# revdotcom/paper_accurate_fast_cheap

Hardware: AMD Instinct MI355X
Metric: audio-sec/sec (1/RTF) GigaSpeech long-form encode (higher is better)
Workload: dtype f32+bf16-slot

## Files before the change

### paper_accurate_fast_cheap_amd/csrc/gemm_ph.hip

```cpp
#include <climits>
#include <cstdlib>
#include <cstring>
#include <type_traits>

#include "pafc_common.h"
#include "../../include/pafc_encoder_ops.h"

namespace pafc {
namespace {

struct PhParams {
    const bf16_t *A, *W;
    const void *bias;
    const void *res;
    void *out;
    long M;
    int N, K;
    long lda, ldw, ldo, ldr;
    long sA, sW, sO, sB, sR;
    float alpha;
    int mtiles, ntiles;
    int tm;
    int batch;
    int nk1, pb_shift;
    long pb_bytes;
    int nsteps, a_lo, w_lo;
    int w_step;
    long lo_off;
    float *ln_stats;
    const float *ln_csum;
    float ln_eps, ln_inv_c;
    int T1, F1, T2, F2, Ci, CiA, CiW, spt, inv_spt;
    long in_bytes;
#ifdef PH_STAMPS
    unsigned long long *stamps;
#endif
};

#ifdef PH_STAMPS
#define PH_STAMP(i) do { if (stamp_on) st[(i)] = __builtin_amdgcn_s_memtime(); } while (0)
#else
#define PH_STAMP(i) do { } while (0)
#endif

__device__ __forceinline__ void dma16(__amdgpu_buffer_rsrc_t rsrc, unsigned lane_off, unsigned uniform_off, void *lds_wave_base) {
    __builtin_amdgcn_raw_ptr_buffer_load_lds(rsrc, (__attribute__((address_space(3))) void *)lds_wave_base, 16, lane_off,
                                             uniform_off, 0, 0);
}
__device__ __forceinline__ __amdgpu_buffer_rsrc_t make_rsrc(const void *base, long bytes) {
    return __builtin_amdgcn_make_buffer_rsrc(const_cast<void *>(base), 0, (int)(bytes > 0x7fffffffL ? 0x7fffffffL : bytes), 0x00020000);
}

#ifndef PH_ST_AUX
#define PH_ST_AUX 0
#endif
#define PH_WAIT(N) asm volatile("s_waitcnt vmcnt(" #N ")" ::: "memory")
template <int N>
__device__ __forceinline__ void wait_vm() {
    static_assert(N >= 0 && N < 64, "vmcnt is a 6-bit counter");
    asm volatile("s_waitcnt vmcnt(%0)" ::"n"(N) : "memory");
}

constexpr int PBN = 256, PBK = 64;
constexpr unsigned PH_OOB = 0xC0000000u;

template <bool GLU, int ACT, int RES, int OUT, bool CONV = false, int LNF = 0, bool SPL = false, bool KSL = false>
__global__ __launch_bounds__(512, 2) void gemm_ph_kernel(const PhParams p) {
    constexpr int BN = PBN;
    constexpr int UA = 128 * 128;
    constexpr int UB = (BN / 2) * 128;
    constexpr int STEP = 2 * UA + 2 * UB;
    constexpr int OFF_A0 = 0, OFF_A1 = UA, OFF_B0 = 2 * UA, OFF_B1 = 2 * UA + UB;
    constexpr int TN = 2;
    constexpr int DA = UA / 8192;
    constexpr int DB = UB / 8192;
    constexpr int OSZ = OUT == 1 ? 4 : 2;
    constexpr bool BIASF32 = OUT != 0;
    constexpr int NST = 8 * (GLU ? 1 : 2) * (OUT == 0 ? 1 : 2) + (LNF == 2 ? 8 : 0);
    static_assert(LNF == 0 || (OUT == 0 && !CONV), "LayerNorm folding: bf16 GEMMs");
    static_assert(!SPL || LNF == 0, "shared-fragment split operands: not with a folded LayerNorm");
    static_assert(LNF != 1 || (RES == 0 && (GLU || ACT == 1)), "LNF 1: the w_1 (SiLU) / pointwise_conv1 (GLU) projections");
    static_assert(LNF != 2 || RES == 1, "LNF 2: a residual GEMM");
    static_assert(!(GLU && (ACT != 0 || RES != 0)), "GLU excludes an activation and a residual");
    static_assert(!(RES != 0 && ACT != 0), "the layer never pairs a residual with an activation");
    static_assert(!KSL || (SPL && !CONV && !GLU && ACT == 0 && RES == 0 && OUT == 1), "K slices: fp32 partial products of split operands");
    extern __shared__ __attribute__((aligned(1024))) unsigned char lds[];

    const int tid = threadIdx.x, lane = tid & 63;
    const int wave = __builtin_amdgcn_readfirstlane(tid >> 6);
    const int wr = wave >> 2, wc = wave & 3;
    const long nblk = (long)p.mtiles * p.ntiles;
    const long total = nblk * p.batch;
    const long per = total / 8;
    const int nt = SPL ? p.nsteps : p.K / PBK;

    auto pix_off = [&](long m) -> long {
        const long tf = (long)p.T2 * p.F2;
        const long bb = m / tf, rem = m - bb * tf;
        const long t2 = rem / p.F2, f2 = rem - t2 * p.F2;
        return (((bb * p.T1 + 2 * t2) * p.F1 + 2 * f2) * p.CiA) * 2;
    };

    struct Tile {
        long m0;
        int n0, z, vr;
        __amdgpu_buffer_rsrc_t Ar, Wr;
    };
    auto make_tile = [&](long t, Tile &T) {
        const bool real = t < total;
        long tt = real ? t : 0;
        if (tt < per * 8) tt = (tt % 8) * per + tt / 8;
        T.z = (int)(tt / nblk);
        const long bid = tt % nblk;
        const int mt0 = (int)(bid / p.ntiles), nt0 = (int)(bid % p.ntiles);
        T.m0 = (long)mt0 * p.tm;
        T.n0 = nt0 * BN;
        T.vr = (int)min((long)p.tm, p.M - T.m0);
        if constexpr (CONV) {
            const long a_base = pix_off(T.m0);
            T.Ar = make_rsrc(reinterpret_cast<const unsigned char *>(p.A) + a_base, real ? p.in_bytes - a_base : 0);
            T.Wr = make_rsrc(p.W + (long)T.n0 * p.CiW, real ? ((long)8 * p.N + p.N - T.n0) * p.CiW * 2 : 0);
        } else {
            T.Ar = make_rsrc(p.A + T.z * p.sA + T.m0 * p.lda, real ? (p.M - T.m0) * p.lda * 2 : 0);
            T.Wr = make_rsrc(p.W + T.z * p.sW + (long)T.n0 * p.ldw, real ? ((long)(p.N - 1 - T.n0) * p.ldw + p.K) * 2 : 0);
        }
    };

    unsigned a_off[2][DA], b_off[2][DB];
    auto a_offsets = [&](const Tile &T, int h) {
        int sl = lane;
        asm volatile("" : "+v"(sl));
        const int sub = sl >> 3, pch = sl & 7;
#pragma unroll
        for (int j = 0; j < DA; ++j) {
            const int u = (wave * DA + j) * 8 + sub;
            const int row = (u >> 6) * 128 + h * 64 + (u & 63);
            const int sc = pch ^ sub;
            const unsigned coff = SPL ? (unsigned)(16 * (sc & 3) + (sc >> 2) * p.a_lo) : (unsigned)(16 * sc);
            a_off[h][j] = CONV ? (unsigned)(pix_off(T.m0 + row) - pix_off(T.m0)) + coff
                               : (unsigned)((long)row * p.lda * 2) + coff;
        }
    };
    auto b_offsets = [&]() {
        const int sub = lane >> 3, pch = lane & 7;
#pragma unroll
        for (int h = 0; h < 2; ++h)
#pragma unroll
            for (int j = 0; j < DB; ++j) {
                const int u = (wave * DB + j) * 8 + sub;
                const int r = u & 31;
                const int pc = ((r & 15) >> 2) * 8 + (r >> 4) * 4 + (r & 3);
                const int sc = pch ^ sub;
                const unsigned coff = SPL ? (unsigned)(16 * (sc & 3) + (sc >> 2) * p.w_lo) : (unsigned)(16 * sc);
                b_off[h][j] = (unsigned)((long)((u >> 5) * 64 + h * 32 + pc) * (CONV ? p.CiW : p.ldw) * 2) + coff;
            }
    };
    auto a_soff = [&](int kt) -> unsigned {
        if constexpr (SPL && !CONV) {
            const int blk = kt >> p.pb_shift, c = kt - (blk << p.pb_shift);
            return (unsigned)(blk * 2 * p.pb_bytes + c * 64);
        } else if constexpr (SPL) {
            const int tap = (kt * p.inv_spt) >> 16, kc = kt - tap * p.spt;
            const int dt = (tap * 11) >> 5, df = tap - 3 * dt;
            return (unsigned)(((dt * p.F1 + df) * p.CiA) * 2 + kc * 64);
        } else if constexpr (!CONV) {
            const int seg = (kt >= p.nk1) + (kt >= 2 * p.nk1);
            const int r = kt - seg * p.nk1;
            const int blk = r >> p.pb_shift, c = r - (blk << p.pb_shift);
            return (unsigned)(blk * 2 * p.pb_bytes + (seg == 1 ? p.pb_bytes : 0) + c * 128);
        } else {
            const int tap = (kt * p.inv_spt) >> 16, kc = kt - tap * p.spt;
            const int seg = (kc >= p.nk1) + (kc >= 2 * p.nk1), cc = kc - seg * p.nk1;
            const int dt = (tap * 11) >> 5, df = tap - 3 * dt;
            return (unsigned)(((dt * p.F1 + df) * p.CiA + (seg == 1 ? p.Ci : 0)) * 2 + cc * 128);
        }
    };
    auto w_soff = [&](int kt) -> unsigned {
        if constexpr (!CONV) return SPL ? kt * p.w_step : kt * 128;
        const int tap = (kt * p.inv_spt) >> 16, kc = kt - tap * p.spt;
        return (unsigned)(tap * p.N * p.CiW * 2 + kc * (SPL ? 64 : 128));
    };
    auto stage_a = [&](const Tile &T, int h, int buf, int kt) {
#ifdef PH_ABL_NODMA
        return;
#endif
        if constexpr (KSL) kt += T.z * nt;
#pragma unroll
        for (int j = 0; j < DA; ++j)
            dma16(T.Ar, a_off[h][j], a_soff(kt), lds + buf * STEP + (h ? OFF_A1 : OFF_A0) + (wave * DA + j) * 1024);
    };
    auto stage_b = [&](const Tile &T, int h, int buf, int kt) {
#ifdef PH_ABL_NODMA
        return;
#endif
        if constexpr (KSL) kt += T.z * nt;
#pragma unroll
        for (int j = 0; j < DB; ++j)
            dma16(T.Wr, b_off[h][j], w_soff(kt), lds + buf * STEP + (h ? OFF_B1 : OFF_B0) + (wave * DB + j) * 1024);
    };

    const int fr = lane & 15, kq = lane >> 4;
    const unsigned frag = fr * 128 + ((kq ^ (fr & 7)) * 16);
    const unsigned la = wr * (64 * 128) + frag;
    const unsigned lb = wc * (32 * 128) + frag;

    bf16x8 af[4][2], bf0[TN][2], bf1[TN][2];
    auto read_a = [&](int h, int buf) {
#ifdef PH_ABL_NOREAD
        return;
#endif
        const unsigned char *base = lds + buf * STEP + (h ? OFF_A1 : OFF_A0);
#pragma unroll
        for (int i = 0; i < 4; ++i) {
            af[i][0] = *reinterpret_cast<const bf16x8 *>(base + la + i * 2048);
            af[i][1] = *reinterpret_cast<const bf16x8 *>(base + (la ^ 64) + i * 2048);
        }
    };
    auto read_b = [&](int h, int buf, bf16x8 (&dst)[TN][2]) {
#ifdef PH_ABL_NOREAD
        return;
#endif
        const unsigned char *base = lds + buf * STEP + (h ? OFF_B1 : OFF_B0);
#pragma unroll
        for (int j = 0; j < TN; ++j) {
            dst[j][0] = *reinterpret_cast<const bf16x8 *>(base + lb + j * 2048);
            dst[j][1] = *reinterpret_cast<const bf16x8 *>(base + (lb ^ 64) + j * 2048);
        }
    };

    Tile cur, nxt;
    make_tile(blockIdx.x, cur);
    a_offsets(cur, 0);
    a_offsets(cur, 1);
    b_offsets();
    stage_a(cur, 0, 0, 0); stage_b(cur, 0, 0, 0); stage_b(cur, 1, 0, 0); stage_a(cur, 1, 0, 0);
    stage_a(cur, 0, 1, 1); stage_b(cur, 0, 1, 1);
    __builtin_amdgcn_sched_barrier(0);
    wait_vm<8>();
    __builtin_amdgcn_sched_barrier(0);
    bool first = true;

    for (long t = blockIdx.x; t < total; t += gridDim.x) {
#ifdef PH_STAMPS
    const bool stamp_on = (wave == 0 || wave == 4) && lane == 0 && cur.z == 0;
    unsigned long long *st = p.stamps + ((size_t)t * 2 + (wave >> 2)) * 64;
    PH_STAMP(0);
#endif
    make_tile(CONV ? total : t + gridDim.x, nxt);
    if constexpr (CONV) {
        if (!first) {
            a_offsets(cur, 0);
            a_offsets(cur, 1);
            stage_a(cur, 0, 0, 0); stage_b(cur, 0, 0, 0); stage_b(cur, 1, 0, 0); stage_a(cur, 1, 0, 0);
            stage_a(cur, 0, 1, 1); stage_b(cur, 0, 1, 1);
            __builtin_amdgcn_sched_barrier(0);
            wait_vm<8>();
            __builtin_amdgcn_sched_barrier(0);
        }
    }
    const bool after_stores = !CONV && !first;
    const bool half_on[2] = {wr * 128 < cur.vr, wr * 128 + 64 < cur.vr};
    constexpr int NBL = LNF == 1 ? 4 : 1;
    {
        const long esz = BIASF32 ? 4 : 2;
        const __amdgpu_buffer_rsrc_t Br = make_rsrc(reinterpret_cast<const unsigned char *>(p.bias) + ((long)cur.z * p.sB + cur.n0) * esz,
                                                    p.bias ? (long)(p.N - cur.n0) * esz : 0);
        dma16(Br, lane * 16, 0, lds + 2 * STEP + wave * 1024);
        if constexpr (LNF == 1) {
            const __amdgpu_buffer_rsrc_t Cr = make_rsrc(p.ln_csum + cur.n0, (long)(p.N - cur.n0) * 4);
            dma16(Cr, lane * 16, 0, lds + 2 * STEP + 8 * 1024 + wave * 1024);
        }
    }

    f32x4 acc[2][2][4][TN];
#pragma unroll
    for (int a = 0; a < 2; ++a)
#pragma unroll
        for (int b = 0; b < 2; ++b)
#pragma unroll
            for (int i = 0; i < 4; ++i)
#pragma unroll
                for (int j = 0; j < TN; ++j) acc[a][b][i][j] = f32x4{0.f, 0.f, 0.f, 0.f};

    auto mma = [&](int mi, int nj, const bf16x8 (&bqf)[TN][2]) {
        __builtin_amdgcn_s_setprio(1);
#ifdef PH_ABL_NOMFMA
        if (false) {
#else
        if (half_on[mi]) {
#endif
            if constexpr (SPL) {
#pragma unroll
                for (int pr = 0; pr < 3; ++pr)
#pragma unroll
                    for (int i = 0; i < 4; ++i)
#pragma unroll
                        for (int j = 0; j < TN; ++j)
                            acc[mi][nj][i][j] = __builtin_amdgcn_mfma_f32_16x16x32_bf16(bqf[j][pr == 2], af[i][pr == 1], acc[mi][nj][i][j], 0, 0, 0);
            } else {
#pragma unroll
                for (int ks = 0; ks < 2; ++ks)
#pragma unroll
                    for (int i = 0; i < 4; ++i)
#pragma unroll
                        for (int j = 0; j < TN; ++j)
                            acc[mi][nj][i][j] = __builtin_amdgcn_mfma_f32_16x16x32_bf16(bqf[j][ks], af[i][ks], acc[mi][nj][i][j], 0, 0, 0);
            }
        }
        __builtin_amdgcn_s_setprio(0);
    };

#ifdef PH_ABL_NOBAR
#define PH_BAR1() do { } while (0)
#else
#define PH_BAR1() __builtin_amdgcn_s_barrier()
#endif
#ifdef PH_ABL_NOEND
#define PH_BAR2() do { } while (0)
#else
#define PH_BAR2() __builtin_amdgcn_s_barrier()
#endif
#define PH_SYNC()                                                                  \
    do {                                                                           \
        if (kt == 0) { if (after_stores) wait_vm<8 + NST + NBL>(); else wait_vm<8 + NBL>(); } \
        else wait_vm<8>();                                                         \
        PH_BAR1();                                                                 \
        __builtin_amdgcn_sched_barrier(0);                                         \
    } while (0)
#define PH_END()                                                                   \
    do {                                                                           \
        __builtin_amdgcn_sched_barrier(0);                                         \
        PH_BAR2();                                                                 \
        __builtin_amdgcn_sched_barrier(0);                                         \
    } while (0)

    auto kstep = [&](auto parc, int kt) {
        constexpr int PAR = decltype(parc)::value;
        const int last = nt - 1 - kt;
        read_b(0, PAR, bf0);
        read_a(0, PAR);
        if (last >= 1) stage_b(cur, 1, PAR ^ 1, kt + 1);
        else stage_b(nxt, 1, PAR ^ 1, 0);
        PH_SYNC();
        mma(0, 0, bf0);
        PH_END();
        read_b(1, PAR, bf1);
        if (last >= 1) stage_a(cur, 1, PAR ^ 1, kt + 1);
        else stage_a(nxt, 1, PAR ^ 1, 0);
        PH_SYNC();
        mma(0, 1, bf1);
        PH_END();
        read_a(1, PAR);
        if (last >= 2) stage_a(cur, 0, PAR, kt + 2);
        else stage_a(nxt, 0, PAR, 1 - last);
        PH_SYNC();
        mma(1, 1, bf1);
        PH_END();
        if (last >= 2) stage_b(cur, 0, PAR, kt + 2);
        else stage_b(nxt, 0, PAR, 1 - last);
        PH_SYNC();
        mma(1, 0, bf0);
        PH_END();
    };
    using I0 = std::integral_constant<int, 0>;
    using I1 = std::integral_constant<int, 1>;

    __builtin_amdgcn_s_barrier();
    if constexpr (LNF == 1) {
        const __amdgpu_buffer_rsrc_t Sd = make_rsrc(p.ln_stats + (cur.z * p.M + cur.m0) * 16, (p.M - cur.m0) * 64);
#pragma unroll
        for (int j = 0; j < 2; ++j)
            dma16(Sd, (wave * 2 + j) * 1024 + lane * 16, 0, lds + 2 * STEP + 16 * 1024 + (wave * 2 + j) * 1024);
    }
    if (wr == 1) __builtin_amdgcn_s_barrier();
    PH_STAMP(1);

    for (int kt = 0; kt < nt; kt += 2) {
        kstep(I0{}, kt);
        PH_STAMP(2 + (kt < 40 ? kt : 40));
        kstep(I1{}, kt + 1);
        PH_STAMP(3 + (kt < 40 ? kt : 40));
    }
    if (wr == 0) __builtin_amdgcn_s_barrier();
    PH_STAMP(50);
#undef PH_SYNC
#undef PH_END

    int etid = tid;
    asm volatile("" : "+v"(etid));
    const int efr = etid & 15, ekq = (etid >> 4) & 3;
    const int ncol = GLU ? p.N / 2 : p.N;
    const int nrt = (cur.vr + 15) >> 4;
    const __amdgpu_buffer_rsrc_t Or = make_rsrc(reinterpret_cast<unsigned char *>(p.out) + (cur.z * p.sO + cur.m0 * p.ldo) * OSZ,
                                                ((p.M - 1 - cur.m0) * p.ldo + (OUT == 2 ? p.lo_off : 0) + ncol) * OSZ);
    constexpr int RSZ = RES == 2 ? 4 : 2;
    __amdgpu_buffer_rsrc_t Rr = Or;
    if constexpr (RES != 0)
        Rr = make_rsrc(reinterpret_cast<const unsigned char *>(p.res) + (cur.z * p.sR + cur.m0 * p.ldr) * RSZ,
                       ((p.M - 1 - cur.m0) * p.ldr + p.N) * RSZ);
    const bool has_bias = p.bias != nullptr;
    auto bias8 = [&](int nj, float (&f)[8]) {
        const unsigned char *slot = lds + 2 * STEP + wave * 1024 + (wc * 64 + nj * 32 + ekq * 8) * (BIASF32 ? 4 : 2);
        if (!has_bias) {
#pragma unroll
            for (int e = 0; e < 8; ++e) f[e] = 0.f;
        } else if constexpr (BIASF32) {
            const u32x4 q0 = *reinterpret_cast<const u32x4 *>(slot), q1 = *reinterpret_cast<const u32x4 *>(slot + 16);
            f[0] = __uint_as_float(q0.x); f[1] = __uint_as_float(q0.y); f[2] = __uint_as_float(q0.z); f[3] = __uint_as_float(q0.w);
            f[4] = __uint_as_float(q1.x); f[5] = __uint_as_float(q1.y); f[6] = __uint_as_float(q1.z); f[7] = __uint_as_float(q1.w);
        } else {
            Elem<bf16_t>::unpack(*reinterpret_cast<const u32x4 *>(slot), f);
        }
    };
    auto store8 = [&](const float (&o)[8], bool live, int row, int col) {
        const bool ok = row < cur.vr && col < ncol;
        const unsigned off = ok ? (unsigned)(((long)row * p.ldo + col) * OSZ) : PH_OOB;
        if constexpr (OUT == 0) {
            u32x4 w{0u, 0u, 0u, 0u};
            if (live) w = u32x4{pack_bf16_rne(o[0], o[1]), pack_bf16_rne(o[2], o[3]), pack_bf16_rne(o[4], o[5]), pack_bf16_rne(o[6], o[7])};
            __builtin_amdgcn_raw_buffer_store_b128(w, Or, off, 0, PH_ST_AUX);
        } else if constexpr (OUT == 1) {
            u32x4 w0{0u, 0u, 0u, 0u}, w1{0u, 0u, 0u, 0u};
            if (live) {
                w0 = u32x4{__float_as_uint(o[0]), __float_as_uint(o[1]), __float_as_uint(o[2]), __float_as_uint(o[3])};
                w1 = u32x4{__float_as_uint(o[4]), __float_as_uint(o[5]), __float_as_uint(o[6]), __float_as_uint(o[7])};
            }
            __builtin_amdgcn_raw_buffer_store_b128(w0, Or, off, 0, PH_ST_AUX);
            __builtin_amdgcn_raw_buffer_store_b128(w1, Or, ok ? off + 16 : PH_OOB, 0, PH_ST_AUX);
        } else {
            u32x4 wh{0u, 0u, 0u, 0u}, wl{0u, 0u, 0u, 0u};
            if (live) {
                float lo[8], hf[8];
                wh = u32x4{pack_bf16_rne(o[0], o[1]), pack_bf16_rne(o[2], o[3]), pack_bf16_rne(o[4], o[5]), pack_bf16_rne(o[6], o[7])};
                Elem<bf16_t>::unpack(wh, hf);
#pragma unroll
                for (int e = 0; e < 8; ++e) lo[e] = o[e] - hf[e];
                wl = u32x4{pack_bf16_rne(lo[0], lo[1]), pack_bf16_rne(lo[2], lo[3]), pack_bf16_rne(lo[4], lo[5]),
                           pack_bf16_rne(lo[6], lo[7])};
            }
            __builtin_amdgcn_raw_buffer_store_b128(wh, Or, off, 0, PH_ST_AUX);
            __builtin_amdgcn_raw_buffer_store_b128(wl, Or, ok ? off + (unsigned)(p.lo_off * 2) : PH_OOB, 0, PH_ST_AUX);
        }
    };
    __amdgpu_buffer_rsrc_t Sr = Or;
    if constexpr (LNF == 2) Sr = make_rsrc(p.ln_stats + (cur.z * p.M + cur.m0) * 16, (p.M - cur.m0) * 64);
    auto row_read = [&](int g, u32x4 (&v)[4]) {
        const unsigned char *rp = lds + 2 * STEP + 16 * 1024 + (wr * 128 + g * 16 + efr) * 64;
#pragma unroll
        for (int q = 0; q < 4; ++q) v[q] = *reinterpret_cast<const u32x4 *>(rp + q * 16);
    };
    auto row_norm = [&](const u32x4 (&v)[4], float &rstd, float &nm) {
        float s1 = 0.f, s2 = 0.f;
#pragma unroll
        for (int q = 0; q < 4; ++q) {
            s1 += __uint_as_float(v[q].x) + __uint_as_float(v[q].z);
            s2 += __uint_as_float(v[q].y) + __uint_as_float(v[q].w);
        }
        const float mean = s1 * p.ln_inv_c;
        const float var = fmaxf(fmaf(-mean, mean, s2 * p.ln_inv_c), 0.f);
        rstd = rsqrtf(var + p.ln_eps);
        nm = -mean * rstd;
    };
    auto csum8 = [&](int nj, float (&f)[8]) {
        const unsigned char *slot = lds + 2 * STEP + 8 * 1024 + wave * 1024 + (wc * 64 + nj * 32 + ekq * 8) * 4;
        const u32x4 q0 = *reinterpret_cast<const u32x4 *>(slot), q1 = *reinterpret_cast<const u32x4 *>(slot + 16);
        f[0] = __uint_as_float(q0.x); f[1] = __uint_as_float(q0.y); f[2] = __uint_as_float(q0.z); f[3] = __uint_as_float(q0.w);
        f[4] = __uint_as_float(q1.x); f[5] = __uint_as_float(q1.y); f[6] = __uint_as_float(q1.z); f[7] = __uint_as_float(q1.w);
    };
    constexpr int RLD = RES == 2 ? 2 : 1;
    float lcs[LNF == 1 ? 2 : 1][8], lbv[LNF == 1 ? 2 : 1][8], nx_rstd = 1.f, nx_nm = 0.f;
    if constexpr (LNF == 1) {
        csum8(0, lcs[0]); csum8(LNF == 1 ? 1 : 0, lcs[LNF == 1 ? 1 : 0]);
        bias8(0, lbv[0]); bias8(LNF == 1 ? 1 : 0, lbv[LNF == 1 ? 1 : 0]);
        u32x4 v0[4];
        row_read(0, v0);
        row_norm(v0, nx_rstd, nx_nm);
    }
    float gst1[LNF == 2 ? 8 : 1], gst2[LNF == 2 ? 8 : 1];
#pragma unroll
    for (int mi = 0; mi < 2; ++mi) {
        u32x4 rr[RES != 0 ? 4 : 1][2][RLD];
        if constexpr (RES != 0) {
            __builtin_amdgcn_sched_barrier(0);
#pragma unroll
            for (int i = 0; i < 4; ++i)
#pragma unroll
                for (int nj = 0; nj < 2; ++nj) {
                    const int row = wr * 128 + mi * 64 + i * 16 + efr, col = cur.n0 + wc * 64 + nj * 32 + ekq * 8;
                    const bool ok = row < cur.vr && col < p.N;
                    const unsigned off = ok ? (unsigned)(((long)row * p.ldr + col) * RSZ) : PH_OOB;
#pragma unroll
                    for (int q = 0; q < RLD; ++q) rr[i][nj][q] = __builtin_amdgcn_raw_buffer_load_b128(Rr, ok ? off + 16 * q : PH_OOB, 0, 0);
                }
        }
#pragma unroll
        for (int i = 0; i < 4; ++i) {
            __builtin_amdgcn_sched_barrier(0);
            const int g = mi * 4 + i;
            const bool live = wr * 8 + g < nrt;
            const int row = wr * 128 + g * 16 + efr;
            const float ln_rstd = nx_rstd, ln_nm = nx_nm;
            u32x4 vn[4];
            if constexpr (LNF == 1) row_read(g < 7 ? g + 1 : 7, vn);
            if constexpr (GLU) {
                float o[8];
                if (live) {
                    float bv[8], bg[8];
                    if constexpr (LNF == 1) {
#pragma unroll
                        for (int e = 0; e < 8; ++e) {
                            bv[e] = fmaf(ln_nm, lcs[0][e], lbv[0][e]);
                            bg[e] = fmaf(ln_nm, lcs[LNF == 1 ? 1 : 0][e], lbv[LNF == 1 ? 1 : 0][e]);
                        }
                    } else {
                        bias8(0, bv);
                        bias8(1, bg);
                    }
                    const float sc = LNF == 1 ? ln_rstd : p.alpha;
#pragma unroll
                    for (int j = 0; j < TN; ++j)
#pragma unroll
                        for (int e = 0; e < 4; ++e) {
                            const float a = fmaf(acc[mi][0][i][j][e], sc, bv[j * 4 + e]);
                            const float b = fmaf(acc[mi][1][i][j][e], sc, bg[j * 4 + e]);
                            o[j * 4 + e] = a * __builtin_amdgcn_rcpf(1.f + __expf(-b));
                        }
                }
                store8(o, live, row, cur.n0 / 2 + wc * 32 + ekq * 8);
            } else {
                float st1 = 0.f, st2 = 0.f;
#pragma unroll
                for (int nj = 0; nj < 2; ++nj) {
                    const int col = cur.n0 + wc * 64 + nj * 32 + ekq * 8;
                    float o[8];
                    if (live) {
                        float bv[8];
                        if constexpr (LNF == 1) {
#pragma unroll
                            for (int e = 0; e < 8; ++e) bv[e] = fmaf(ln_nm, lcs[LNF == 1 ? nj : 0][e], lbv[LNF == 1 ? nj : 0][e]);
                        } else {
                            bias8(nj, bv);
                        }
                        const float sc = LNF == 1 ? ln_rstd : p.alpha;
#pragma unroll
                        for (int j = 0; j < TN; ++j)
#pragma unroll
                            for (int e = 0; e < 4; ++e)
                                o[j * 4 + e] = epilogue_act<ACT>(fmaf(acc[mi][nj][i][j][e], sc, bv[j * 4 + e]));
                        if constexpr (RES == 1) {
                            float rv[8];
                            Elem<bf16_t>::unpack(rr[i][nj][0], rv);
#pragma unroll
                            for (int e = 0; e < 8; ++e) o[e] += rv[e];
                        } else if constexpr (RES == 2) {
                            o[0] += __uint_as_float(rr[i][nj][0].x); o[1] += __uint_as_float(rr[i][nj][0].y);
                            o[2] += __uint_as_float(rr[i][nj][0].z); o[3] += __uint_as_float(rr[i][nj][0].w);
                            o[4] += __uint_as_float(rr[i][nj][RLD - 1].x); o[5] += __uint_as_float(rr[i][nj][RLD - 1].y);
                            o[6] += __uint_as_float(rr[i][nj][RLD - 1].z); o[7] += __uint_as_float(rr[i][nj][RLD - 1].w);
                        }
                        if constexpr (LNF == 2) {
                            float q[8];
                            Elem<bf16_t>::unpack(u32x4{pack_bf16_rne(o[0], o[1]), pack_bf16_rne(o[2], o[3]), pack_bf16_rne(o[4], o[5]),
                                                       pack_bf16_rne(o[6], o[7])}, q);
#pragma unroll
                            for (int e = 0; e < 8; ++e) { st1 += q[e]; st2 = fmaf(q[e], q[e], st2); }
                        }
                    }
                    store8(o, live, row, col);
                }
                if constexpr (LNF == 2) { gst1[LNF == 2 ? g : 0] = live ? st1 : 0.f; gst2[LNF == 2 ? g : 0] = live ? st2 : 0.f; }
            }
            if constexpr (LNF == 1) row_norm(vn, nx_rstd, nx_nm);
        }
    }
    if constexpr (LNF == 2) {
        __builtin_amdgcn_sched_barrier(0);
#pragma unroll
        for (int g = 0; g < 8; ++g) { gst1[g] += __shfl_xor(gst1[g], 16, 64); gst2[g] += __shfl_xor(gst2[g], 16, 64); }
#pragma unroll
        for (int g = 0; g < 8; ++g) { gst1[g] += __shfl_xor(gst1[g], 32, 64); gst2[g] += __shfl_xor(gst2[g], 32, 64); }
#pragma unroll
        for (int g = 0; g < 8; ++g) {
            const int row = wr * 128 + g * 16 + efr;
            const bool ok = ekq == 0 && row < cur.vr;
            const unsigned off = ok ? (unsigned)(row * 64 + ((cur.n0 >> 8) * 4 + wc) * 8) : PH_OOB;
            __builtin_amdgcn_raw_buffer_store_b64(u32x2{__float_as_uint(gst1[g]), __float_as_uint(gst2[g])}, Sr, off, 0, 0);
        }
    }
    __builtin_amdgcn_sched_barrier(0);
    first = false;
    if constexpr (CONV) make_tile(t + gridDim.x, cur);
    else cur = nxt;
    PH_STAMP(53);
    }
    PH_WAIT(0);
}

__global__ __launch_bounds__(256) void gemm_ph_ktail_fixup_kernel(const float *__restrict__ part, long slab, int kslices,
                                                                  const float *__restrict__ bias, const float *res, long ldr,
                                                                  float *out, long ldo, long rows, int N, float alpha) {
    const int nq = N >> 2;
    const long total = rows * nq;
    for (long i = (long)blockIdx.x * blockDim.x + threadIdx.x; i < total; i += (long)gridDim.x * blockDim.x) {
        const long m = i / nq;
        const int n = (int)(i - m * nq) << 2;
        float4 acc = *reinterpret_cast<const float4 *>(part + m * N + n);
        for (int z = 1; z < kslices; ++z) {
            const float4 q = *reinterpret_cast<const float4 *>(part + z * slab + m * N + n);
            acc.x += q.x; acc.y += q.y; acc.z += q.z; acc.w += q.w;
        }
        float4 b = make_float4(0.f, 0.f, 0.f, 0.f);
        if (bias) b = *reinterpret_cast<const float4 *>(bias + n);
        float4 o = make_float4(fmaf(acc.x, alpha, b.x), fmaf(acc.y, alpha, b.y), fmaf(acc.z, alpha, b.z), fmaf(acc.w, alpha, b.w));
        if (res) {
            const float4 r = *reinterpret_cast<const float4 *>(res + m * ldr + n);
            o.x += r.x; o.y += r.y; o.z += r.z; o.w += r.w;
        }
        *reinterpret_cast<float4 *>(out + m * ldo + n) = o;
    }
}

template <bool GLU, int ACT, int RES, int OUT, bool CONV = false, int LNF = 0, bool SPL = false, bool KSL = false>
int launch_ph(const PhParams &p, int batch, hipStream_t s) {
    constexpr size_t lds = 2 * (2 * 128 * 128 + 2 * (PBN / 2) * 128) + 8 * 1024 + (LNF == 1 ? 8 * 1024 + 16 * 1024 : 0);
    auto kern = gemm_ph_kernel<GLU, ACT, RES, OUT, CONV, LNF, SPL, KSL>;
    static bool attr_set[64];
    int dev = 0;
    if (hipGetDevice(&dev) != hipSuccess) return PAFC_ERR_LAUNCH;
    if (dev < 0 || dev >= 64 || !attr_set[dev]) {
        if (hipFuncSetAttribute((const void *)kern, hipFuncAttributeMaxDynamicSharedMemorySize, (int)lds) != hipSuccess)
            return PAFC_ERR_LAUNCH;
        if (dev >= 0 && dev < 64) attr_set[dev] = true;
    }
    const int cus = device_cus();
    PhParams q = p;
    q.batch = batch;
    const long total = (long)p.mtiles * p.ntiles * batch;
    const long grid = total < cus ? total : cus;
    hipLaunchKernelGGL(kern, dim3((unsigned)grid), dim3(512), lds, s, q);
    return hipGetLastError() == hipSuccess ? PAFC_OK : PAFC_ERR_LAUNCH;
}

int g_split_walk = -1;
bool split_shared_fragments() {
    if (g_split_walk < 0) {
        const char *e = getenv("PAFC_SPLIT_WALK");
        g_split_walk = !(e && std::strcmp(e, "hilohi") == 0);
    }
    return g_split_walk != 0;
}

}
}

extern "C" int pafc_gemm_ph_ex(long M, int N, int K, int batch, const void *A, long lda, long strideA, int a_split, const void *W,
                               long ldw, long strideW, const void *bias, long strideBias, const void *residual, int res_kind,
                               long ldr, long strideR, void *out, int out_kind, long ldo, long lo_off, long strideO, float alpha,
                               int act, int tile_m, pafc_stream_t stream) {
    return pafc_gemm_ph_ex2(M, N, K, batch, A, lda, strideA, a_split, 0, W, ldw, strideW, bias, strideBias, residual, res_kind, ldr,
                            strideR, out, out_kind, ldo, lo_off, strideO, alpha, act, tile_m, stream);
}

extern "C" int pafc_gemm_ph_ex2(long M, int N, int K, int batch, const void *A, long lda, long strideA, int a_split,
                                int a_plane_block, const void *W, long ldw, long strideW, const void *bias, long strideBias,
                                const void *residual, int res_kind, long ldr, long strideR, void *out, int out_kind, long ldo,
                                long lo_off, long strideO, float alpha, int act, int tile_m, pafc_stream_t stream) {
    if (!A || !W || !out) return PAFC_ERR_NULL_POINTER;
    if (M <= 0 || N <= 0 || K <= 0 || batch <= 0 || batch > 65535) return PAFC_ERR_BAD_DIMS;
    if (act < 0 || act > 4 || out_kind < 0 || out_kind > 2 || res_kind < 0 || res_kind > 2) return PAFC_ERR_UNSUPPORTED;
    if (!residual) res_kind = 0;
    else if (res_kind == 0) return PAFC_ERR_BAD_DIMS;
    const bool glu = act == 4;
    if (tile_m < 64 || tile_m > 256 || tile_m % 64) return PAFC_ERR_UNSUPPORTED;
    if (N % 8 || K % 128) return PAFC_ERR_UNSUPPORTED;
    if (glu && (N % 256 || residual)) return PAFC_ERR_UNSUPPORTED;
    if (residual && act != 0) return PAFC_ERR_UNSUPPORTED;
    if (res_kind == 1 && out_kind != 0) return PAFC_ERR_UNSUPPORTED;
    if (res_kind == 2 && out_kind != 1) return PAFC_ERR_UNSUPPORTED;
    const int Kw = a_split ? 3 * K : K;
    const int No = glu ? N / 2 : N;
    if (lda < (a_split ? 2 * K : K) || ldw < Kw || (residual && ldr < N)) return PAFC_ERR_BAD_DIMS;
    if (out_kind == 2 ? (lo_off < No || ldo < lo_off + No) : ldo < No) return PAFC_ERR_BAD_DIMS;
    if ((lda | ldw | strideA | strideW) % 8 || (ldo | strideO | lo_off) % 8 || (residual && ((ldr | strideR) % 8))) return PAFC_ERR_ALIGNMENT;
    if ((((uintptr_t)A | (uintptr_t)W | (uintptr_t)out | (uintptr_t)residual | (uintptr_t)bias) & 15) != 0) return PAFC_ERR_ALIGNMENT;
    if ((double)M * lda * 2 >= 2.0e9 || (double)N * ldw * 2 >= 2.0e9) return PAFC_ERR_UNSUPPORTED;
    if ((double)256 * ldo * 4 >= 2.0e9 || (residual && (double)256 * ldr * 4 >= 2.0e9)) return PAFC_ERR_UNSUPPORTED;
    pafc::PhParams p{};
    p.A = (const pafc::bf16_t *)A; p.W = (const pafc::bf16_t *)W; p.bias = bias; p.res = residual; p.out = out;
    p.M = M; p.N = N; p.K = Kw;
    p.lda = lda; p.ldw = ldw; p.ldo = ldo; p.ldr = ldr;
    p.sA = strideA; p.sW = strideW; p.sO = strideO; p.sB = strideBias; p.sR = strideR;
    p.alpha = alpha;
    p.nk1 = a_split ? K / 64 : INT_MAX / 4;
    p.pb_shift = 31;
    p.pb_bytes = (long)K * 2;
    if (a_split && a_plane_block) {
        int sh = 0;
        while ((64 << sh) < a_plane_block) ++sh;
        if ((64 << sh) != a_plane_block || K % a_plane_block) return PAFC_ERR_UNSUPPORTED;
        p.pb_shift = sh;
        p.pb_bytes = (long)a_plane_block * 2;
    }
    p.lo_off = lo_off;
    p.tm = tile_m;
    p.mtiles = (int)((M + tile_m - 1) / tile_m);
    p.ntiles = (N + 255) / 256;
    if ((long)p.mtiles * p.ntiles > 0x7fffffffL) return PAFC_ERR_BAD_DIMS;
    hipStream_t s = (hipStream_t)stream;
    if (a_split && out_kind != 0 && pafc::split_shared_fragments() && (double)2 * K * 2 + 64 < 2.0e9) {
        p.nsteps = K / 32;
        p.a_lo = (int)p.pb_bytes;
        p.w_lo = 2 * K * 2;
        p.w_step = 64;
        p.pb_shift = p.pb_shift >= 30 ? 30 : p.pb_shift + 1;
        if (out_kind == 1) {
            if (glu) return pafc::launch_ph<true, 0, 0, 1, false, 0, true>(p, batch, s);
            if (res_kind == 2) return pafc::launch_ph<false, 0, 2, 1, false, 0, true>(p, batch, s);
            if (act == 0) return pafc::launch_ph<false, 0, 0, 1, false, 0, true>(p, batch, s);
            return PAFC_ERR_UNSUPPORTED;
        }
        if (glu || residual) return PAFC_ERR_UNSUPPORTED;
        if (act == 1) return pafc::launch_ph<false, 1, 0, 2, false, 0, true>(p, batch, s);
        if (act == 0) return pafc::launch_ph<false, 0, 0, 2, false, 0, true>(p, batch, s);
        return PAFC_ERR_UNSUPPORTED;
    }
    if (out_kind == 0) {
        if (glu) return pafc::launch_ph<true, 0, 0, 0>(p, batch, s);
        if (res_kind == 1) return pafc::launch_ph<false, 0, 1, 0>(p, batch, s);
        switch (act) {
            case 1: return pafc::launch_ph<false, 1, 0, 0>(p, batch, s);
            case 2: return pafc::launch_ph<false, 2, 0, 0>(p, batch, s);
            case 3: return pafc::launch_ph<false, 3, 0, 0>(p, batch, s);
            default: return pafc::launch_ph<false, 0, 0, 0>(p, batch, s);
        }
    }
    if (out_kind == 1) {
        if (glu) return pafc::launch_ph<true, 0, 0, 1>(p, batch, s);
        if (res_kind == 2) return pafc::launch_ph<false, 0, 2, 1>(p, batch, s);
        if (act == 0) return pafc::launch_ph<false, 0, 0, 1>(p, batch, s);
        return PAFC_ERR_UNSUPPORTED;
    }
    if (glu || residual) return PAFC_ERR_UNSUPPORTED;
    if (act == 1) return pafc::launch_ph<false, 1, 0, 2>(p, batch, s);
    if (act == 0) return pafc::launch_ph<false, 0, 0, 2>(p, batch, s);
    return PAFC_ERR_UNSUPPORTED;
}

extern "C" int pafc_gemm_bf16_ph_ln(long M, int N, int K, const void *A, long lda, const void *W, long ldw, const void *bias,
                                    const void *residual, long ldr, void *out, long ldo, float alpha, int act, int ln_mode,
                                    float *stats, const float *csum, int ln_c, float ln_eps, int tile_m, pafc_stream_t stream) {
    if (!A || !W || !out || !stats) return PAFC_ERR_NULL_POINTER;
    if (M <= 0 || N <= 0 || K <= 0 || ln_c <= 0) return PAFC_ERR_BAD_DIMS;
    if (tile_m < 64 || tile_m > 256 || tile_m % 64) return PAFC_ERR_UNSUPPORTED;
    if (N % 8 || K % 128) return PAFC_ERR_UNSUPPORTED;
    const bool glu = act == 4;
    if (ln_mode == 1) {
        if (!csum || residual || (act != 1 && act != 4) || alpha != 1.f || K != ln_c) return PAFC_ERR_UNSUPPORTED;
        if (glu && N % 256) return PAFC_ERR_UNSUPPORTED;
    } else if (ln_mode == 2) {
        if (!residual || act != 0 || N != 512 || ln_c != N) return PAFC_ERR_UNSUPPORTED;
    } else {
        return PAFC_ERR_UNSUPPORTED;
    }
    const int No = glu ? N / 2 : N;
    if (lda < K || ldw < K || ldo < No || (residual && ldr < N)) return PAFC_ERR_BAD_DIMS;
    if ((lda | ldw | ldo) % 8 || (residual && ldr % 8)) return PAFC_ERR_ALIGNMENT;
    if ((((uintptr_t)A | (uintptr_t)W | (uintptr_t)out | (uintptr_t)residual | (uintptr_t)bias | (uintptr_t)stats | (uintptr_t)csum) & 15) != 0)
        return PAFC_ERR_ALIGNMENT;
    if ((double)M * lda * 2 >= 2.0e9 || (double)N * ldw * 2 >= 2.0e9 || (double)256 * ldo * 4 >= 2.0e9 ||
        (residual && (double)256 * ldr * 4 >= 2.0e9))
        return PAFC_ERR_UNSUPPORTED;
    pafc::PhParams p{};
    p.A = (const pafc::bf16_t *)A; p.W = (const pafc::bf16_t *)W; p.bias = bias; p.res = residual; p.out = out;
    p.M = M; p.N = N; p.K = K;
    p.lda = lda; p.ldw = ldw; p.ldo = ldo; p.ldr = ldr;
    p.alpha = alpha;
    p.nk1 = INT_MAX / 4; p.pb_shift = 31; p.pb_bytes = (long)K * 2;
    p.ln_stats = stats; p.ln_csum = csum; p.ln_eps = ln_eps; p.ln_inv_c = 1.f / (float)ln_c;
    p.tm = tile_m;
    p.mtiles = (int)((M + tile_m - 1) / tile_m);
    p.ntiles = (N + 255) / 256;
    if ((long)p.mtiles * p.ntiles > 0x7fffffffL) return PAFC_ERR_BAD_DIMS;
    hipStream_t s = (hipStream_t)stream;
    if (ln_mode == 2) return pafc::launch_ph<false, 0, 1, 0, false, 2>(p, 1, s);
    if (glu) return pafc::launch_ph<true, 0, 0, 0, false, 1>(p, 1, s);
    return pafc::launch_ph<false, 1, 0, 0, false, 1>(p, 1, s);
}

extern "C" int pafc_gemm_bf16_ph(long M, int N, int K, int batch, const void *A, long lda, long strideA, const void *W,
                                 long ldw, long strideW, const void *bias, long strideBias, const void *residual, long ldr,
                                 long strideR, void *out, long ldo, long strideO, float alpha, int act, int tile_n,
                                 int tile_m, pafc_stream_t stream) {
    if (tile_n != 256) return PAFC_ERR_UNSUPPORTED;
    return pafc_gemm_ph_ex(M, N, K, batch, A, lda, strideA, 0, W, ldw, strideW, bias, strideBias, residual, residual ? 1 : 0, ldr,
                           strideR, out, 0, ldo, 0, strideO, alpha, act, tile_m, stream);
}

static int conv_ph_launch(int B, int T1, int F1, int Ci, int Co, const void *in, const void *w, const void *bias, void *out,
                          int relu, int tile_m, int split, pafc_stream_t stream) {
    if (!in || !w || !out) return PAFC_ERR_NULL_POINTER;
    if (B <= 0 || T1 < 3 || F1 < 3 || Ci <= 0 || Co <= 0) return PAFC_ERR_BAD_DIMS;
    if (Ci % 128 || Co % 8) return PAFC_ERR_UNSUPPORTED;
    if (tile_m != 256 && tile_m != 192 && tile_m != 128) return PAFC_ERR_UNSUPPORTED;
    if ((((uintptr_t)in | (uintptr_t)w | (uintptr_t)out | (uintptr_t)bias) & 15) != 0) return PAFC_ERR_ALIGNMENT;
    const int T2 = (T1 - 3) / 2 + 1, F2 = (F1 - 3) / 2 + 1;
    const long M = (long)B * T2 * F2;
    pafc::PhParams p{};
    p.A = (const pafc::bf16_t *)in; p.W = (const pafc::bf16_t *)w; p.bias = bias; p.out = out;
    p.Ci = Ci; p.CiA = split ? 2 * Ci : Ci; p.CiW = split ? 3 * Ci : Ci;
    if ((double)9 * Co * p.CiW * 2 >= 2.0e9 || (double)3 * F1 * p.CiA * 2 >= 2.0e9) return PAFC_ERR_UNSUPPORTED;
    p.M = M; p.N = Co; p.K = 9 * p.CiW; p.lda = p.CiA; p.ldw = p.CiW; p.alpha = 1.f;
    p.ldo = split ? 2 * Co : Co; p.lo_off = split ? Co : 0;
    p.nk1 = Ci / 64;
    p.pb_shift = 31; p.pb_bytes = 0;
    p.spt = p.CiW / 64;
    p.inv_spt = (65536 + p.spt - 1) / p.spt;
    for (int kt = 0; kt < p.K / 64 + 2; ++kt)
        if (((kt * p.inv_spt) >> 16) != kt / p.spt) return PAFC_ERR_UNSUPPORTED;
    p.T1 = T1; p.F1 = F1; p.T2 = T2; p.F2 = F2;
    p.in_bytes = (long)B * T1 * F1 * p.CiA * 2;
    p.tm = tile_m;
    p.mtiles = (int)((M + tile_m - 1) / tile_m);
    p.ntiles = (Co + 255) / 256;
    hipStream_t s = (hipStream_t)stream;
    if (split && pafc::split_shared_fragments()) {
        p.spt = Ci / 32;
        p.inv_spt = (65536 + p.spt - 1) / p.spt;
        p.nsteps = 9 * p.spt;
        for (int kt = 0; kt < p.nsteps + 2; ++kt)
            if (((kt * p.inv_spt) >> 16) != kt / p.spt) return PAFC_ERR_UNSUPPORTED;
        p.a_lo = Ci * 2;
        p.w_lo = 2 * Ci * 2;
        return relu ? pafc::launch_ph<false, 3, 0, 2, true, 0, true>(p, 1, s) : pafc::launch_ph<false, 0, 0, 2, true, 0, true>(p, 1, s);
    }
    if (split) return relu ? pafc::launch_ph<false, 3, 0, 2, true>(p, 1, s) : pafc::launch_ph<false, 0, 0, 2, true>(p, 1, s);
    return relu ? pafc::launch_ph<false, 3, 0, 0, true>(p, 1, s) : pafc::launch_ph<false, 0, 0, 0, true>(p, 1, s);
}

extern "C" int pafc_conv3x3s2_nhwc_bf16_ph(int B, int T1, int F1, int Ci, int Co, const void *in, const void *w_tap_co_ci,
                                           const void *bias, void *out, int relu, int tile_m, pafc_stream_t stream) {
    return conv_ph_launch(B, T1, F1, Ci, Co, in, w_tap_co_ci, bias, out, relu, tile_m, 0, stream);
}

extern "C" int pafc_conv3x3s2_nhwc_split_ph(int B, int T1, int F1, int Ci, int Co, const void *in_planes, const void *w3_tap_co_3ci,
                                            const float *bias, void *out_planes, int relu, int tile_m, pafc_stream_t stream) {
    return conv_ph_launch(B, T1, F1, Ci, Co, in_planes, w3_tap_co_3ci, bias, out_planes, relu, tile_m, 1, stream);
}

extern "C" int pafc_gemm_ph_ktail(long M, int N, int K, int batch, const void *A, long lda, long strideA, int a_split,
                                  int a_plane_block, const void *W, long ldw, long strideW, const void *bias, long strideBias,
                                  const void *residual, int res_kind, long ldr, long strideR, void *out, int out_kind, long ldo,
                                  long lo_off, long strideO, float alpha, int act, int tile_m, void *workspace,
                                  size_t workspace_bytes, long split_row, int kslices, pafc_stream_t stream) {
    if (!A || !W || !out || !workspace) return PAFC_ERR_NULL_POINTER;
    if (M <= 0 || N <= 0 || K <= 0) return PAFC_ERR_BAD_DIMS;
    if (act < 0 || act > 4 || out_kind < 0 || out_kind > 2 || res_kind < 0 || res_kind > 2) return PAFC_ERR_UNSUPPORTED;
    if (!a_split || out_kind != 1 || act != 0 || batch != 1 || tile_m != 256 || kslices != 2) return PAFC_ERR_UNSUPPORTED;
    if (!pafc::split_shared_fragments()) return PAFC_ERR_UNSUPPORTED;
    if (!residual) res_kind = 0;
    else if (res_kind == 0) return PAFC_ERR_BAD_DIMS;
    else if (res_kind != 2) return PAFC_ERR_UNSUPPORTED;
    if (split_row < 0 || split_row >= M || split_row % 256) return PAFC_ERR_BAD_DIMS;
    if (K % (64 * kslices)) return PAFC_ERR_BAD_DIMS;
    if (N % 8) return PAFC_ERR_UNSUPPORTED;
    const long rows = M - split_row;
    if (workspace_bytes < (size_t)kslices * (size_t)rows * (size_t)N * sizeof(float)) return PAFC_ERR_BAD_DIMS;
    if (lda < 2 * (long)K || ldw < 3 * (long)K || (residual && ldr < N) || ldo < N) return PAFC_ERR_BAD_DIMS;
    if ((lda | ldw) % 8 || ldo % 8 || (residual && ldr % 8)) return PAFC_ERR_ALIGNMENT;
    if ((((uintptr_t)A | (uintptr_t)W | (uintptr_t)out | (uintptr_t)residual | (uintptr_t)bias | (uintptr_t)workspace) & 15) != 0)
        return PAFC_ERR_ALIGNMENT;
    if ((double)M * lda * 2 >= 2.0e9 || (double)N * ldw * 2 >= 2.0e9 || (double)2 * K * 2 + 64 >= 2.0e9) return PAFC_ERR_UNSUPPORTED;
    if ((double)256 * ldo * 4 >= 2.0e9 || (residual && (double)256 * ldr * 4 >= 2.0e9)) return PAFC_ERR_UNSUPPORTED;
    int pb_shift = 30;
    long pb_bytes = (long)K * 2;
    if (a_plane_block) {
        int sh = 0;
        while ((64 << sh) < a_plane_block) ++sh;
        if ((64 << sh) != a_plane_block || K % a_plane_block) return PAFC_ERR_UNSUPPORTED;
        pb_shift = sh + 1;
        pb_bytes = (long)a_plane_block * 2;
    }
    hipStream_t s = (hipStream_t)stream;
    if (split_row > 0) {
        const int rc = pafc_gemm_ph_ex2(split_row, N, K, 1, A, lda, strideA, 1, a_plane_block, W, ldw, strideW, bias, strideBias,
                                        residual, res_kind, ldr, strideR, out, 1, ldo, lo_off, strideO, alpha, 0, 256, stream);
        if (rc != PAFC_OK) return rc;
    }
    pafc::PhParams p{};
    p.A = (const pafc::bf16_t *)A + split_row * lda; p.W = (const pafc::bf16_t *)W; p.out = workspace;
    p.M = rows; p.N = N; p.K = 3 * K;
    p.lda = lda; p.ldw = ldw; p.ldo = N;
    p.sO = rows * N;
    p.alpha = 1.f;
    p.nk1 = K / 64;
    p.pb_shift = pb_shift;
    p.pb_bytes = pb_bytes;
    p.nsteps = K / 32 / kslices;
    p.a_lo = (int)pb_bytes;
    p.w_lo = 2 * K * 2;
    p.w_step = 64;
    p.tm = 256;
    p.mtiles = (int)((rows + 255) / 256);
    p.ntiles = (N + 255) / 256;
    const int rc = pafc::launch_ph<false, 0, 0, 1, false, 0, true, true>(p, kslices, s);
    if (rc != PAFC_OK) return rc;
    const long quads = rows * (N / 4);
    const long cap = (long)pafc::device_cus() * 32;
    const long blocks = (quads + 255) / 256;
    hipLaunchKernelGGL(pafc::gemm_ph_ktail_fixup_kernel, dim3((unsigned)(blocks < cap ? blocks : cap)), dim3(256), 0, s,
                       (const float *)workspace, rows * N, kslices, (const float *)bias,
                       residual ? (const float *)residual + split_row * ldr : nullptr, ldr, (float *)out + split_row * ldo, ldo, rows, N,
                       alpha);
    return hipGetLastError() == hipSuccess ? PAFC_OK : PAFC_ERR_LAUNCH;
}
```

Measured before the change: 48550.

## Store GEMM epilogue as whole 128-byte row lines via DPP lane swaps

Adds a store-variant template parameter to the persistent GEMM kernel. Adjacent row lanes exchange halves with a DPP quad swap so that each lane writes a contiguous 32-byte piece and the wave covers whole 128-byte lines of a row. An optional nontemporal cache policy is used for some forms. A table selects the variant per GEMM form when the output is 128-byte aligned, and an environment variable can force a choice. The aim is fewer partial cache-line writes, at the cost of extra DPP and select instructions plus more template instantiations.

```diff
diff --git a/paper_accurate_fast_cheap_amd/csrc/gemm_ph.hip b/paper_accurate_fast_cheap_amd/csrc/gemm_ph.hip
--- a/paper_accurate_fast_cheap_amd/csrc/gemm_ph.hip
+++ b/paper_accurate_fast_cheap_amd/csrc/gemm_ph.hip
@@ -64,7 +64,7 @@
 constexpr int PBN = 256, PBK = 64;
 constexpr unsigned PH_OOB = 0xC0000000u;
 
-template <bool GLU, int ACT, int RES, int OUT, bool CONV = false, int LNF = 0, bool SPL = false, bool KSL = false>
+template <bool GLU, int ACT, int RES, int OUT, bool CONV = false, int LNF = 0, bool SPL = false, bool KSL = false, int ST = 0>
 __global__ __launch_bounds__(512, 2) void gemm_ph_kernel(const PhParams p) {
     constexpr int BN = PBN;
     constexpr int UA = 128 * 128;
@@ -84,6 +84,8 @@
     static_assert(!(GLU && (ACT != 0 || RES != 0)), "GLU excludes an activation and a residual");
     static_assert(!(RES != 0 && ACT != 0), "the layer never pairs a residual with an activation");
     static_assert(!KSL || (SPL && !CONV && !GLU && ACT == 0 && RES == 0 && OUT == 1), "K slices: fp32 partial products of split operands");
+    static_assert(ST == 0 || (LNF == 0 && OUT != 2 && !(GLU && OUT == 0)), "whole-line stores: bf16 / fp32 forms whose waves own 128 bytes of a row");
+    constexpr int AUX = ST == 2 ? 2 : PH_ST_AUX;
     extern __shared__ __attribute__((aligned(1024))) unsigned char lds[];
 
     const int tid = threadIdx.x, lane = tid & 63;
@@ -442,6 +444,32 @@
             __builtin_amdgcn_raw_buffer_store_b128(wl, Or, ok ? off + (unsigned)(p.lo_off * 2) : PH_OOB, 0, PH_ST_AUX);
         }
     };
+    const int eodd = efr & 1;
+    auto pack8 = [&](const float (&o)[8], bool live, u32x4 &q0, u32x4 &q1) {
+        q0 = u32x4{0u, 0u, 0u, 0u};
+        q1 = u32x4{0u, 0u, 0u, 0u};
+        if (!live) return;
+        if constexpr (OUT == 1) {
+            q0 = u32x4{__float_as_uint(o[0]), __float_as_uint(o[1]), __float_as_uint(o[2]), __float_as_uint(o[3])};
+            q1 = u32x4{__float_as_uint(o[4]), __float_as_uint(o[5]), __float_as_uint(o[6]), __float_as_uint(o[7])};
+        } else {
+            q0 = u32x4{pack_bf16_rne(o[0], o[1]), pack_bf16_rne(o[2], o[3]), pack_bf16_rne(o[4], o[5]), pack_bf16_rne(o[6], o[7])};
+        }
+    };
+    auto swap1 = [&](unsigned v) -> unsigned {
+        return (unsigned)__builtin_amdgcn_mov_dpp((int)v, 0xB1, 0xF, 0xF, true);
+    };
+    auto store_pair = [&](const u32x4 &a, const u32x4 &b, int row, unsigned posA, unsigned posB, bool cokA, bool cokB) {
+        const u32x4 na{swap1(a.x), swap1(a.y), swap1(a.z), swap1(a.w)}, nb{swap1(b.x), swap1(b.y), swap1(b.z), swap1(b.w)};
+        u32x4 s0, s1;
+        s0.x = eodd ? nb.x : a.x; s0.y = eodd ? nb.y : a.y; s0.z = eodd ? nb.z : a.z; s0.w = eodd ? nb.w : a.w;
+        s1.x = eodd ? b.x : na.x; s1.y = eodd ? b.y : na.y; s1.z = eodd ? b.z : na.z; s1.w = eodd ? b.w : na.w;
+        const int re = row & ~1;
+        const bool cok = eodd ? cokB : cokA;
+        const unsigned off0 = (unsigned)((long)re * p.ldo * OSZ) + (eodd ? posB : posA);
+        __builtin_amdgcn_raw_buffer_store_b128(s0, Or, cok && re < cur.vr ? off0 : PH_OOB, 0, AUX);
+        __builtin_amdgcn_raw_buffer_store_b128(s1, Or, cok && re + 1 < cur.vr ? off0 + (unsigned)(p.ldo * OSZ) : PH_OOB, 0, AUX);
+    };
     __amdgpu_buffer_rsrc_t Sr = Or;
     if constexpr (LNF == 2) Sr = make_rsrc(p.ln_stats + (cur.z * p.M + cur.m0) * 16, (p.M - cur.m0) * 64);
     auto row_read = [&](int g, u32x4 (&v)[4]) {
@@ -526,9 +554,17 @@
                             o[j * 4 + e] = a * __builtin_amdgcn_rcpf(1.f + __expf(-b));
                         }
                 }
-                store8(o, live, row, cur.n0 / 2 + wc * 32 + ekq * 8);
+                if constexpr (ST == 0) {
+                    store8(o, live, row, cur.n0 / 2 + wc * 32 + ekq * 8);
+                } else {
+                    const int col = cur.n0 / 2 + wc * 32 + ekq * 8;
+                    u32x4 q0, q1;
+                    pack8(o, live, q0, q1);
+                    store_pair(q0, q1, row, (unsigned)col * 4, (unsigned)col * 4 + 16, col < ncol, col < ncol);
+                }
             } else {
                 float st1 = 0.f, st2 = 0.f;
+                u32x4 pk[ST != 0 ? 2 : 1][2];
 #pragma unroll
                 for (int nj = 0; nj < 2; ++nj) {
                     const int col = cur.n0 + wc * 64 + nj * 32 + ekq * 8;
@@ -566,7 +602,18 @@
                             for (int e = 0; e < 8; ++e) { st1 += q[e]; st2 = fmaf(q[e], q[e], st2); }
                         }
                     }
-                    store8(o, live, row, col);
+                    if constexpr (ST == 0) {
+                        store8(o, live, row, col);
+                    } else {
+                        pack8(o, live, pk[ST != 0 ? nj : 0][0], pk[ST != 0 ? nj : 0][1]);
+                        if constexpr (OUT == 1)
+                            store_pair(pk[ST != 0 ? nj : 0][0], pk[ST != 0 ? nj : 0][1], row, (unsigned)col * 4, (unsigned)col * 4 + 16,
+                                       col < ncol, col < ncol);
+                    }
+                }
+                if constexpr (ST != 0 && OUT == 0) {
+                    const int col = cur.n0 + wc * 64 + ekq * 8;
+                    store_pair(pk[0][0], pk[ST != 0 ? 1 : 0][0], row, (unsigned)col * 2, (unsigned)col * 2 + 64, col < ncol, col + 32 < ncol);
                 }
                 if constexpr (LNF == 2) { gst1[LNF == 2 ? g : 0] = live ? st1 : 0.f; gst2[LNF == 2 ? g : 0] = live ? st2 : 0.f; }
             }
@@ -620,10 +667,10 @@
     }
 }
 
-template <bool GLU, int ACT, int RES, int OUT, bool CONV = false, int LNF = 0, bool SPL = false, bool KSL = false>
-int launch_ph(const PhParams &p, int batch, hipStream_t s) {
+template <bool GLU, int ACT, int RES, int OUT, bool CONV, int LNF, bool SPL, bool KSL, int ST>
+int launch_ph_st(const PhParams &p, int batch, hipStream_t s) {
     constexpr size_t lds = 2 * (2 * 128 * 128 + 2 * (PBN / 2) * 128) + 8 * 1024 + (LNF == 1 ? 8 * 1024 + 16 * 1024 : 0);
-    auto kern = gemm_ph_kernel<GLU, ACT, RES, OUT, CONV, LNF, SPL, KSL>;
+    auto kern = gemm_ph_kernel<GLU, ACT, RES, OUT, CONV, LNF, SPL, KSL, ST>;
     static bool attr_set[64];
     int dev = 0;
     if (hipGetDevice(&dev) != hipSuccess) return PAFC_ERR_LAUNCH;
@@ -639,6 +686,46 @@
     const long grid = total < cus ? total : cus;
     hipLaunchKernelGGL(kern, dim3((unsigned)grid), dim3(512), lds, s, q);
     return hipGetLastError() == hipSuccess ? PAFC_OK : PAFC_ERR_LAUNCH;
+}
+
+constexpr bool ph_store_variants(bool GLU, int ACT, int RES, int OUT, bool CONV, int LNF, bool SPL, bool KSL) {
+    if (CONV || LNF != 0 || ACT != 0 || KSL) return false;
+    if (SPL && GLU && OUT == 1) return true;
+    if (SPL && !GLU && RES == 2 && OUT == 1) return true;
+    if (SPL && !GLU && RES == 0 && OUT == 1) return true;
+    if (!SPL && !GLU && RES == 0 && OUT == 0) return true;
+    if (!SPL && !GLU && RES == 2 && OUT == 1) return true;
+    return false;
+}
+constexpr int ph_store_table(bool GLU, int ACT, int RES, int OUT, bool CONV, int LNF, bool SPL, bool KSL, bool lined, int K) {
+    if (!ph_store_variants(GLU, ACT, RES, OUT, CONV, LNF, SPL, KSL)) return 0;
+    if (SPL && GLU) return lined ? 2 : 0;
+    if (SPL && RES == 2) return lined && K <= 3 * 1024 ? 2 : 0;
+    if (SPL) return lined ? 0 : 1;
+    if (OUT == 0) return lined ? 1 : 0;
+    return lined ? 2 : 0;
+}
+int ph_store_forced() {
+    const char *e = getenv("PAFC_PH_STORE");
+    if (!e) return -1;
+    if (std::strcmp(e, "legacy") == 0) return 0;
+    if (std::strcmp(e, "lines") == 0) return 1;
+    if (std::strcmp(e, "lines_nt") == 0) return 2;
+    return -1;
+}
+
+template <bool GLU, int ACT, int RES, int OUT, bool CONV = false, int LNF = 0, bool SPL = false, bool KSL = false>
+int launch_ph(const PhParams &p, int batch, hipStream_t s) {
+    if constexpr (ph_store_variants(GLU, ACT, RES, OUT, CONV, LNF, SPL, KSL)) {
+        const long osz = OUT == 1 ? 4 : 2;
+        const bool lined = ((uintptr_t)p.out & 127) == 0 && (p.ldo * osz) % 128 == 0 && (batch == 1 || (p.sO * osz) % 128 == 0) &&
+                           p.N % 64 == 0;
+        int st = ph_store_forced();
+        if (st < 0) st = ph_store_table(GLU, ACT, RES, OUT, CONV, LNF, SPL, KSL, lined, p.K);
+        if (st == 1) return launch_ph_st<GLU, ACT, RES, OUT, CONV, LNF, SPL, KSL, 1>(p, batch, s);
+        if (st == 2) return launch_ph_st<GLU, ACT, RES, OUT, CONV, LNF, SPL, KSL, 2>(p, batch, s);
+    }
+    return launch_ph_st<GLU, ACT, RES, OUT, CONV, LNF, SPL, KSL, 0>(p, batch, s);
 }
 
 int g_split_walk = -1;
```

New measurement: 48970 (median of 5 runs). No clear change (+0.9%).
